# UniBwTAS/continuous_clustering

Hardware: AMD Instinct MI355X
Metric: Mpoints/s clustered (64-beam streams) (higher is better)
Workload: dtype f32

## Files before the change

### continuous_clustering_amd/csrc/cc_k_segment.h

```cpp
#pragma once


template<int RPL>
__device__ __forceinline__ void table_scan_tiles(const SP& p, const int R, const int ntiles, const int lane)
{
    float carry[RPL];
#pragma unroll
    for (int k = 0; k < RPL; k++)
    {
        const int row = k * 64 + lane;
        carry[k] = row < R ? p.curtab[row] : 0.f;
    }
    constexpr int U = 8;
    for (int t0 = 0; t0 < ntiles; t0 += U)
    {
        float v[U][RPL];
#pragma unroll
        for (int u = 0; u < U; u++)
#pragma unroll
            for (int k = 0; k < RPL; k++)
            {
                const int row = k * 64 + lane;
                v[u][k] = (row < R && t0 + u < ntiles) ? p.tabc[(size_t) (t0 + u) * R + row] : __builtin_nanf("");
            }
#pragma unroll
        for (int u = 0; u < U; u++)
#pragma unroll
            for (int k = 0; k < RPL; k++)
            {
                const int row = k * 64 + lane;
                if (row < R && t0 + u < ntiles)
                {
                    p.tabc[(size_t) (t0 + u) * R + row] = carry[k];
                    if (!(v[u][k] != v[u][k]))
                        carry[k] = v[u][k];
                }
            }
    }
#pragma unroll
    for (int k = 0; k < RPL; k++)
    {
        const int row = k * 64 + lane;
        if (row < R)
            p.curtab[row] = carry[k];
    }
}

template<int RPL>
__global__ __launch_bounds__(64 * TABLE_WAVES) void k_table(Geometry g, Planes P, StreamState* states, int first_stream, int slot)
{
    const int s = first_stream + blockIdx.x;
    const int lane = lane_id(), wave = uniform_i32((int) (threadIdx.x >> 6));
    StreamState* st = &states[s];
#ifdef CC_CHAIN2_PRIO
    __builtin_amdgcn_s_setprio(CC_CHAIN2_PRIO);
#endif
    if (threadIdx.x == 0)
        st->batch[slot].mode = st->assoc_mode;
    const long long seg_begin = st->batch[slot].seg_begin, seg_end = st->batch[slot].seg_end;
    if (seg_begin < 0 || seg_begin >= seg_end)
        return;
    if (st->batch[slot].fused)
        return;
    const SP p = stream_ptrs(P, g, s);
    const int R = g.num_rows, RC = g.ring_cols;
    const int ntiles = (int) ((seg_end - seg_begin + 63) >> 6);
    constexpr int U = 16;
    for (int t = wave; t < ntiles; t += TABLE_WAVES)
    {
        const long long c_lo = seg_begin + 64ll * t, c_hi = (c_lo + 64 < seg_end ? c_lo + 64 : seg_end);
        float last[RPL];
#pragma unroll
        for (int k = 0; k < RPL; k++)
            last[k] = __builtin_nanf("");
        int lc = (int) (c_lo % RC);
        for (long long c0 = c_lo; c0 < c_hi; c0 += U)
        {
            float cur[U][RPL], below[U][RPL];
#pragma unroll
            for (int u = 0; u < U; u++)
            {
#pragma unroll
                for (int k = 0; k < RPL; k++)
                {
                    const int row = k * 64 + lane;
                    cur[u][k] = below[u][k] = 0.f;
                    if (row < R && c0 + u < c_hi)
                    {
                        const size_t ci = (size_t) lc * R + row;
                        cur[u][k] = p.incl[ci];
                        below[u][k] = row + 1 < R ? p.incl[ci + 1] : 0.f;
                    }
                }
                lc = lc + 1 == RC ? 0 : lc + 1;
            }
#pragma unroll
            for (int u = 0; u < U; u++)
            {
                if (c0 + u >= c_hi)
                    break;
#pragma unroll
                for (int k = 0; k < RPL; k++)
                {
                    const float diff = cur[u][k] - below[u][k];
                    if (!(diff != diff))
                        last[k] = diff;
                }
            }
        }
#pragma unroll
        for (int k = 0; k < RPL; k++)
        {
            const int row = k * 64 + lane;
            if (row < R)
                p.tabc[(size_t) t * R + row] = last[k];
        }
    }
    __syncthreads();
    if (wave == 0)
        table_scan_tiles<RPL>(p, R, ntiles, lane);
}

__device__ __forceinline__ void ego_record(const StreamState* __restrict__ states, int first_stream, const cc_config& cfg, const double* __restrict__ poses,
                                           long long n, long long n_total, long long fbase, double* __restrict__ out, const int sl, const long long f)
{
    const double* A = states[first_stream + sl].robot_from_sensor;
    const double* T = poses + ((size_t) sl * (size_t) n_total + (size_t) fbase + (size_t) f) * 12;
    double ir[9], it[3];
    for (int i = 0; i < 3; i++)
        for (int j = 0; j < 3; j++)
            ir[i * 3 + j] = T[j * 4 + i];
    for (int i = 0; i < 3; i++)
        it[i] = ((-ir[i * 3 + 0]) * T[3] + (-ir[i * 3 + 1]) * T[7]) + (-ir[i * 3 + 2]) * T[11];
    double* o = out + ((size_t) sl * (size_t) n + (size_t) f) * EGO_STRIDE;
    for (int i = 0; i < 3; i++)
    {
        for (int j = 0; j < 3; j++)
            o[i * 3 + j] = (A[i * 4 + 0] * ir[0 * 3 + j] + A[i * 4 + 1] * ir[1 * 3 + j]) + A[i * 4 + 2] * ir[2 * 3 + j];
        o[9 + i] = ((A[i * 4 + 0] * it[0] + A[i * 4 + 1] * it[1]) + A[i * 4 + 2] * it[2]) + A[i * 4 + 3];
    }
    auto gram_dev = [](const double* m, const int stride) -> double
    {
        double dev = 0.;
        for (int a = 0; a < 3; a++)
            for (int b = 0; b < 3; b++)
            {
                double d = 0.;
                for (int k = 0; k < 3; k++)
                    d += m[k * stride + a] * m[k * stride + b];
                d -= a == b ? 1. : 0.;
                dev += d * d;
            }
        return __builtin_sqrt(dev);
    };
    const double dev_t = gram_dev(T, 4), dev_a = gram_dev(A, 4);
    auto mx2 = [](const float a, const float b) -> double
    {
        const double x = a, y = b;
        return x * x > y * y ? x * x : y * y;
    };
    const double box = __builtin_sqrt(mx2(cfg.length_ref_to_front_end_, cfg.length_ref_to_rear_end_) + mx2(cfg.width_ref_to_left_mirror_, cfg.width_ref_to_right_mirror_) +
                                      mx2(cfg.height_ref_to_maximum_, cfg.height_ref_to_ground_));
    const double at = __builtin_sqrt((A[3] * A[3] + A[7] * A[7]) + A[11] * A[11]);
    double skip = __builtin_inf();
    if (dev_t < 0.5 && dev_a < 0.5 && box == box && at == at)
    {
        const double sigma = __builtin_sqrt((1. - dev_t) * (1. - dev_a));
        const double delta = 2.4e-7 * ((__builtin_fabs(T[3]) + __builtin_fabs(T[7])) + __builtin_fabs(T[11])) + 1e-6;
        const double r = ((box + at) / sigma + delta) * 1.00001;
        const double r2 = r * r * 1.00001;
        float r2f = (float) r2;
        if ((double) r2f < r2)
            r2f = __builtin_bit_cast(float, __builtin_bit_cast(int, r2f) + 1);
        skip = r2f == r2f ? (double) r2f : __builtin_inf();
    }
    o[12] = skip;
}

__global__ __launch_bounds__(256) void k_ego(const StreamState* __restrict__ states, int first_stream, cc_config cfg, const double* __restrict__ poses,
                                             long long n, long long n_total, long long fbase, double* __restrict__ out)
{
    const long long f = (long long) blockIdx.x * 256 + threadIdx.x;
    if (f < n)
        ego_record(states, first_stream, cfg, poses, n, n_total, fbase, out, (int) blockIdx.y, f);
}


template<int RPL>
__global__ __launch_bounds__(64) void k_seg_pre(Geometry g, cc_config cfg, Planes P, StreamState* states, int first_stream, int slot,
                                                const double* __restrict__ poses, long long n_total, long long fbase,
                                                const double* __restrict__ ego, long long n_batch)
{
    const int sl = blockIdx.x;
    const int s = first_stream + sl;
    StreamState* st = &states[s];
    const long long seg_begin = st->batch[slot].seg_begin, seg_end = st->batch[slot].seg_end;
    if (seg_begin < 0 || seg_begin >= seg_end)
        return;
    if (st->batch[slot].fused)
        return;
    if (!st->has_robot_tf)
    {
        if (blockIdx.y == 0 && lane_id() == 0)
            raise_error(st, CC_ERR_NO_ROBOT_TRANSFORM, seg_begin, 0);
        return;
    }
    const SP p = stream_ptrs(P, g, s);
    const int R = g.num_rows, RC = g.ring_cols;
    const int lane = lane_id();

    const long long total = seg_end - seg_begin;
    const long long chunk_len = (total + SEGPRE_BLOCKS - 1) / SEGPRE_BLOCKS;
    const long long c_lo = seg_begin + chunk_len * (long long) blockIdx.y, c_hi = (c_lo + chunk_len < seg_end ? c_lo + chunk_len : seg_end);
    if (c_lo >= c_hi)
        return;
    const int NC = g.num_columns;
    int lc = (int) (c_lo % RC);
    long long rot = c_lo / NC;
    int cir = (int) (c_lo - rot * NC);
    long long pass = c_lo / RC;
    uint16_t a_tg[RPL];
    uint16_t n_tg[RPL];
    float n_dist[RPL], n_incaz[RPL];
    float4 n_rec[RPL];
    uint8_t n_inten[RPL];
    int n_trig = 0;
    auto load_tags = [&](const long long gcx, const int lcx)
    {
#pragma unroll
        for (int k = 0; k < RPL; k++)
        {
            const int row = k * 64 + lane;
            a_tg[k] = CELL_CLEARED;
            if (row < R && gcx < c_hi)
                a_tg[k] = p.gtag[(size_t) lcx * R + row];
        }
    };
    auto load_cells = [&](const long long gcx, const int lcx, const uint16_t tagx)
    {
#pragma unroll
        for (int k = 0; k < RPL; k++)
        {
            const int row = k * 64 + lane;
            n_dist[k] = n_incaz[k] = 0.f;
            n_inten[k] = 0;
            n_rec[k] = make_float4(__builtin_nanf(""), __builtin_nanf(""), __builtin_nanf(""), __builtin_nanf(""));
            if (row < R && gcx < c_hi)
            {
                const size_t ci = (size_t) lcx * R + row;
                n_dist[k] = p.dist[ci];
                if (n_tg[k] == tagx)
                {
                    n_rec[k] = p.sc_rec[ci];
                    n_incaz[k] = p.incaz[ci];
                    n_inten[k] = p.inten[ci];
                }
            }
        }
        if (gcx < c_hi)
            n_trig = p.trig[lcx];
    };
    load_tags(c_lo, lc);
    CazBase cb = caz_base_of_rotation(rot);
    long long cb_rot = rot;
    for (long long gc = c_lo; gc < c_hi; gc++, pass += (lc + 1 == RC ? 1 : 0), lc = (lc + 1 == RC ? 0 : lc + 1), rot += (cir + 1 == NC ? 1 : 0),
                   cir = (cir + 1 == NC ? 0 : cir + 1))
    {
        const size_t base = (size_t) lc * R;
        if (rot != cb_rot)
        {
            cb = caz_base_of_rotation(rot);
            cb_rot = rot;
        }
        const uint16_t tag = cell_tag(pass);
        {
#pragma unroll
            for (int k = 0; k < RPL; k++)
                n_tg[k] = a_tg[k];
            load_cells(gc, lc, tag);
            load_tags(gc + 1, lc + 1 == RC ? 0 : lc + 1);
        }
        const int trig = uniform_i32(n_trig);
        const double* T = poses + ((size_t) sl * (size_t) n_total + (size_t) fbase + (size_t) trig) * 12;
        const double* E = ego + ((size_t) sl * (size_t) n_batch + (size_t) trig) * EGO_STRIDE;
        const float spx = (float) T[3], spy = (float) T[7], spz = (float) T[11];

        float cx[RPL], cy[RPL], cz[RPL], dist[RPL], incl[RPL];
        bool empty_cell[RPL], overrun = false;
        int overrun_row = -1;
        long long overrun_gcol = -1;
#pragma unroll
        for (int k = 0; k < RPL; k++)
        {
            const int row = k * 64 + lane;
            dist[k] = incl[k] = __builtin_nanf("");
            cx[k] = cy[k] = cz[k] = 0.f;
            empty_cell[k] = false;
            if (row < R)
            {
                const uint16_t tg = n_tg[k];
                if (tg != tag && tg != CELL_CLEARED)
                {
                    overrun = true;
                    overrun_row = row;
                    overrun_gcol = gc - (long long) ((((unsigned) tag - (unsigned) tg) & 0x7fffu)) * RC;
                }
                empty_cell[k] = tg != tag;
                dist[k] = n_dist[k];
                cx[k] = n_rec[k].x;
                cy[k] = n_rec[k].y;
                cz[k] = n_rec[k].z;
                incl[k] = n_rec[k].w;
            }
        }
        if (__any(overrun))
        {
            const int worst = -wave_min_i32(-overrun_row);
            if (overrun_row == worst)
            {
                atomicMin((unsigned long long*) &st->overrun_col, (unsigned long long) gc);
                raise_error(st, CC_ERR_RING_OVERRUN, overrun_gcol, gc);
            }
            continue;
        }
        float x2[RPL], uz[RPL], w[RPL];
        int flags[RPL];
        seg_pre_cells<RPL>(cfg, R, lane, cx, cy, cz, dist, incl, n_inten, spx, spy, spz, E, x2, uz, w, flags);
        int kpos = 0x7fffffff, kneg = 0x7fffffff;
        bool any_empty = false;
#pragma unroll
        for (int k = 0; k < RPL; k++)
        {
            const int row = k * 64 + lane;
            if (row >= R)
                continue;
            const size_t ci = base + row;
            if (empty_cell[k])
                p.gtag[ci] = tag;
            if (flags[k] & SG_NAN)
                any_empty = true;
            else
                caz_key(n_incaz[k], kpos, kneg);
            p.sg_x2[ci] = x2[k];
            p.sg_uz[ci] = uz[k];
            p.sg_w[ci] = w[k];
            p.sg_flags[ci] = (uint8_t) flags[k];
        }
        const double min_az = column_min_caz(cb, kpos, kneg, any_empty, gc, g.az_width);
        if (lane == 0)
        {
            p.colg[lc] = gc;
            p.colminaz[lc] = min_az;
        }
    }
}

#ifndef CC_SEGSCAN_MIN_WAVES_PER_SIMD
#define CC_SEGSCAN_MIN_WAVES_PER_SIMD 2
#endif
constexpr int SEG_X2_RING = 16;
constexpr int SEG_CH = 16;
constexpr int SEG_FEW = 4;
__host__ __device__ inline int seg_pitch_f(int R)
{
    (void) R;
    return SEG_X2_RING + 1;
}
__host__ __device__ inline int seg_pitch_b(int R)
{
    return ((R + 3) & ~3) + 4;
}
__host__ __device__ inline bool seg_tiled(int R)
{
    return R >= SEG_CH && (R % SEG_CH) == 0;
}
__host__ inline size_t seg_scan_lds_bytes(int R)
{
    const size_t f = seg_tiled(R) ? (size_t) 4 * 64 * SEG_CH * 4 : (size_t) 64 * seg_pitch_f(R) * 4;
    return f + (size_t) 64 * seg_pitch_b(R);
}

enum
{
    SG_G_UNKNOWN = 0, SG_G_GROUND = 1, SG_G_OBSTACLE = 2, SG_G_EGO = 3, SG_G_FOG = 4,
    SG_D_WHITE = 0, SG_D_GRAY = 1, SG_D_ORANGE = 2, SG_D_GREEN = 3, SG_D_YELLOWGREEN = 4, SG_D_YELLOW = 5, SG_D_RED = 6, SG_D_DARKRED = 7,
    SG_D_VIOLET = 8, SG_D_LIGHTGRAY = 9
};

__global__ __launch_bounds__(64, CC_SEGSCAN_MIN_WAVES_PER_SIMD) void k_seg_scan(Geometry g, cc_config cfg, Planes P, StreamState* states, int first_stream, int slot)
{
    const int s = first_stream + blockIdx.x;
    StreamState* st = &states[s];
    const long long seg_begin = st->batch[slot].seg_begin, seg_end = st->batch[slot].seg_end;
    if (seg_begin < 0 || st->error != 0)
        return;
    const long long tile0 = seg_begin + (long long) blockIdx.y * 64;
    if (tile0 >= seg_end)
        return;
    const int ncols = (int) (seg_end - tile0 < 64 ? seg_end - tile0 : 64);
    const SP p = stream_ptrs(P, g, s);
    const int R = g.num_rows, RC = g.ring_cols;
    const int lane = lane_id();
    const int PF = seg_pitch_f(R), PB = seg_pitch_b(R);
    const bool tiled = seg_tiled(R);
    extern __shared__ __attribute__((aligned(16))) unsigned char smem[];
    float* l_x2 = (float*) smem;
    unsigned char* l_out = (unsigned char*) (l_x2 + (tiled ? 4 * 64 * SEG_CH : 64 * PF));

    const int lc0 = (int) (tile0 % RC);
    {
        const bool active = lane < ncols;
        const long long gc = tile0 + lane;
        int lcl = lc0 + lane;
        lcl = lcl >= RC ? lcl - RC : lcl;
        const float* gx = p.sg_x2 + (size_t) lcl * R;
        const float* gz = p.sg_uz + (size_t) lcl * R;
        const float* gw = p.sg_w + (size_t) lcl * R;
        const unsigned char* gf = p.sg_flags + (size_t) lcl * R;
        float4* g_rec = p.sc_rec + (size_t) lcl * R;
        float* g_incl = p.incl + (size_t) lcl * R;
        const float* tab_in = p.tabc + (size_t) blockIdx.y * R;
        unsigned char* oo = l_out + lane * PB;
        const float height_sensor_to_ground = -(float) st->robot_from_sensor[11] + cfg.height_ref_to_ground_;
        const bool chess_odd = cfg.ignore_points_in_chessboard_pattern && (gc & 1);
        const bool chess_even = cfg.ignore_points_in_chessboard_pattern && !(gc & 1);
        bool first_obstacle_detected = false, first_point_found = false;
        float lg2x = 0.f, lgz = height_sensor_to_ground;
        float pv2x = 0.f, pvz = 0.f;
        unsigned char previous_label = 0;
        auto row_step = [&](const int row, const int f, const float cur2x, const float cur2y, auto&& x2_below)
        {
            const bool valid = (f & (SG_NAN | SG_FOG | SG_EGO)) == 0;
            const bool first = valid & !first_point_found;
            const bool normal = valid & first_point_found;
            const bool ign = ((f & (SG_TOO_CLOSE | SG_INCL_IGNORE)) != 0) | ((row & 1) ? chess_even : chess_odd);
            const float h = cur2y - height_sensor_to_ground;
            const bool first_ground = (h > cfg.first_ring_as_ground_min_allowed_z_diff) & (h < cfg.first_ring_as_ground_max_allowed_z_diff);
            const float p2cx = cur2x - pv2x, p2cy = cur2y - pvz;
            const float slope_to_prev = p2cy / p2cx;
            const bool flat_prev = (ccm::absf(slope_to_prev) < cfg.max_slope) & (p2cx > 0) & ((cfg.use_terrain == 0) | (p2cx < 5));
            const float l2cx = cur2x - lg2x, l2cy = cur2y - lgz;
            const float slope_to_lg = l2cy / l2cx;
            const bool flat_lg = (ccm::absf(slope_to_lg) < cfg.max_slope) & (l2cx > 0);
            const bool no_terrain = cfg.use_terrain == 0;
            const bool green = !first_obstacle_detected & flat_prev;
            const bool yellowgreen = !green & no_terrain & first_obstacle_detected & flat_prev & flat_lg;
            const bool yellow = !green & !yellowgreen & no_terrain &
                                (ccm::absf(l2cx) < cfg.ground_because_close_to_last_certain_ground_max_dist_diff) &
                                (ccm::absf(l2cy) < cfg.ground_because_close_to_last_certain_ground_max_z_diff);
            const bool ground_n = green | yellowgreen | yellow;
            const unsigned d_n = green ? (unsigned) SG_D_GREEN : (yellowgreen ? (unsigned) SG_D_YELLOWGREEN : (yellow ? (unsigned) SG_D_YELLOW : (unsigned) SG_D_RED));
            const unsigned g_n = ground_n ? (unsigned) SG_G_GROUND : (unsigned) SG_G_OBSTACLE;
            const unsigned d_f = first_ground ? (unsigned) SG_D_GRAY : (unsigned) SG_D_ORANGE;
            const unsigned g_f = first_ground ? (unsigned) SG_G_GROUND : (unsigned) SG_G_OBSTACLE;
            unsigned g = first ? g_f : g_n, d = first ? d_f : d_n;
            g = (f & SG_EGO) ? (unsigned) SG_G_EGO : g;
            d = (f & SG_EGO) ? (unsigned) SG_D_VIOLET : d;
            g = (f & SG_FOG) ? (unsigned) SG_G_FOG : g;
            d = (f & SG_FOG) ? (unsigned) SG_D_LIGHTGRAY : d;
            g = (f & SG_NAN) ? (unsigned) SG_G_UNKNOWN : g;
            d = (f & SG_NAN) ? (unsigned) SG_D_WHITE : d;
            const bool red = normal & !ground_n;
            if (__any(red))
            {
                int below = row + 1;
                bool go = red & (below < R);
                while (__any(go))
                {
                    const int bi = go ? below : row + 1 < R ? row + 1 : row;
                    const unsigned bo = oo[bi];
                    const unsigned bg = bo & 7u, bd = (bo >> 3) & 15u;
                    const float xb = x2_below(bi, go);
                    const bool is_ground = bg == (unsigned) SG_G_GROUND;
                    const bool cont = go & ((bd == (unsigned) SG_D_YELLOW) |
                                            (is_ground & (ccm::absf(cur2x - xb) < cfg.obstacle_because_next_certain_obstacle_max_dist_diff)));
                    if (cont & is_ground)
                        oo[bi] = (unsigned char) ((bo & 0x80u) | SG_G_OBSTACLE | (SG_D_DARKRED << 3));
                    below += cont ? 1 : 0;
                    go = cont & (below < R);
                }
            }
            first_obstacle_detected = first ? !first_ground : (first_obstacle_detected | red);
            const bool keep_as_ground = normal & (green | yellowgreen) & (slope_to_prev > cfg.last_ground_point_slope_higher_than) &
                                        (ccm::absf(p2cx) < cfg.last_ground_point_distance_smaller_than) & (previous_label != SG_D_YELLOW);
            const bool new_lg = (first & first_ground) | keep_as_ground;
            lg2x = new_lg ? cur2x : lg2x;
            lgz = new_lg ? cur2y : lgz;
            pv2x = valid ? cur2x : pv2x;
            pvz = valid ? cur2y : pvz;
            previous_label = valid ? (unsigned char) d : previous_label;
            first_point_found |= valid;
            oo[row] = (unsigned char) (g | (d << 3) | ((valid & ign) ? 0x80u : 0u));
        };
        const unsigned long long le_mask = lane == 63 ? ~0ull : ((2ull << lane) - 1ull);
        const bool supplement = cfg.supplement_inclination_angle_for_nan_cells != 0;
        const bool step_filter = cfg.ignore_points_with_too_big_inclination_angle_diff != 0;
        float supp_below = __builtin_nanf("");
        bool below_nan = false;
        auto row_all = [&](const int row, const int f, const float cur2x, const float cur2y, const float wv, const float carry, auto&& x2_below,
                           auto&& stash) -> bool
        {
            const bool own = !(f & (SG_NAN | SG_PENDING));
            const unsigned long long m = __ballot(own) & le_mask;
            const int src = m ? 63 - __clzll((long long) m) : lane;
            const float got = __shfl(wv, src, 64);
            const float tab = m ? got : carry;
            const bool is_nan = (f & SG_NAN) != 0;
            const float supp = (supplement & (row < R - 1)) ? (below_nan ? supp_below : wv) + tab : __builtin_nanf("");
            if (is_nan & active)
            {
                g_rec[row] = make_float4(__builtin_nanf(""), __builtin_nanf(""), __builtin_nanf(""), supp);
                g_incl[row] = supp;
            }
            supp_below = is_nan ? supp : supp_below;
            below_nan = is_nan;
            const bool pend = ((f & (SG_PENDING | SG_NAN)) == SG_PENDING) & step_filter & (row < R - 1) & !(tab != tab);
            const float a = wv * tab;
            const bool in_range = (cfg.max_distance > 0.f) & (tab >= 0.f) & (tab < 0.05f) & (wv > 0.f) & (wv < 3.0e38f);
            const bool surely_not = in_range & (cfg.max_distance >= 1.01f * a);
            const bool surely = in_range & !surely_not & (cfg.max_distance * 1.000002f < a);
            const int fx = f | ((pend & surely) ? SG_INCL_IGNORE : 0);
            const bool need = pend & !surely_not & !surely;
            if (need)
                stash(tab);
            row_step(row, fx, cur2x, cur2y, x2_below);
            return need;
        };
        if (tiled && ncols <= SEG_FEW && 3 * SEG_FEW * R <= 4 * 64 * SEG_CH)
        {
            float* cx2 = l_x2;
            float* cuz = l_x2 + SEG_FEW * R;
            float* cw = l_x2 + 2 * SEG_FEW * R;
            for (int c = 0; c < ncols; c++)
            {
                int l = lc0 + c;
                l = l >= RC ? l - RC : l;
                for (int row = lane; row < R; row += 64)
                {
                    cx2[c * R + row] = p.sg_x2[(size_t) l * R + row];
                    cuz[c * R + row] = p.sg_uz[(size_t) l * R + row];
                    cw[c * R + row] = p.sg_w[(size_t) l * R + row];
                    l_out[c * PB + row] = p.sg_flags[(size_t) l * R + row];
                }
            }
            wave_lds_fence();
            asm volatile("s_waitcnt lgkmcnt(0)" ::: "memory");
            {
                const int lc_ = active ? lane : 0;
                const float* mx = cx2 + lc_ * R;
                const float* mz = cuz + lc_ * R;
                const float* mw = cw + lc_ * R;
                auto x2_below = [&](const int below, const bool wanted) -> float { (void) wanted; return mx[below]; };
                const float carry_lo = lane < R ? tab_in[lane] : 0.f, carry_hi = 64 + lane < R ? tab_in[64 + lane] : 0.f;
                auto carry_of = [&](const int row) -> float
                {
                    return __builtin_bit_cast(float, __builtin_amdgcn_readlane(__builtin_bit_cast(int, row < 64 ? carry_lo : carry_hi), row & 63));
                };
                for (int b = R - 4; b >= 0; b -= 4)
                {
                    const float4 a = *(const float4*) (mx + b);
                    const float4 c4 = *(const float4*) (mz + b);
                    const float4 w4 = *(const float4*) (mw + b);
                    const float x4[4] = {a.x, a.y, a.z, a.w}, z4[4] = {c4.x, c4.y, c4.z, c4.w}, ww[4] = {w4.x, w4.y, w4.z, w4.w};
                    const unsigned fw = active ? *(const unsigned*) (oo + b) : 0x01010101u * (unsigned) SG_NAN;
                    unsigned pend = 0;
#pragma unroll
                    for (int u = 3; u >= 0; u--)
                        if (row_all(b + u, (int) ((fw >> (8 * u)) & 0xffu), x4[u], z4[u], ww[u], carry_of(b + u), x2_below,
                                    [&](const float tab) { cuz[lc_ * R + b + u] = tab; }))
                            pend |= 1u << u;
                    if (__any(pend != 0))
                        for (int u = 0; u < 4; u++)
                            if (((pend >> u) & 1) && ccm::atan2f_exact(cfg.max_distance, mw[b + u]) < mz[b + u])
                                oo[b + u] |= 0x80;
                }
            }
        }
        else if (tiled)
        {
            float* t_uz = l_x2 + 2 * 64 * SEG_CH;
            float* t_w = l_x2 + 3 * 64 * SEG_CH;
            const int ld_c = lane >> 2, ld_q = lane & 3;
            int ld_off[4];
#pragma unroll
            for (int j = 0; j < 4; j++)
            {
                const int c = j * 16 + ld_c;
                int l = lc0 + c;
                l = l >= RC ? l - RC : l;
                ld_off[j] = c < ncols ? l * R : -1;
            }
            float4 nx[4], nz[4], nw[4];
            float ncarry = 0.f;
            auto load_chunk = [&](const int b)
            {
                ncarry = tab_in[b + (lane & 15)];
#pragma unroll
                for (int j = 0; j < 4; j++)
                {
                    nx[j] = nz[j] = nw[j] = make_float4(0.f, 0.f, 0.f, 0.f);
                    if (ld_off[j] >= 0)
                    {
                        nx[j] = *(const float4*) (p.sg_x2 + (size_t) ld_off[j] + b + ld_q * 4);
                        nz[j] = *(const float4*) (p.sg_uz + (size_t) ld_off[j] + b + ld_q * 4);
                        nw[j] = *(const float4*) (p.sg_w + (size_t) ld_off[j] + b + ld_q * 4);
                    }
                }
            };
            int b = R - SEG_CH;
            load_chunk(b);
            {
                const int npieces = R >> 4;
                for (int idx0 = lane; idx0 < 64 * npieces; idx0 += 4 * 64)
                {
                    uint4 v[4];
                    int dst[4];
#pragma unroll
                    for (int u = 0; u < 4; u++)
                    {
                        const int idx = idx0 + u * 64;
                        const int c = idx / npieces, piece = idx - c * npieces;
                        dst[u] = -1;
                        v[u] = make_uint4(0, 0, 0, 0);
                        if (idx < 64 * npieces && c < ncols)
                        {
                            int l = lc0 + c;
                            l = l >= RC ? l - RC : l;
                            v[u] = *(const uint4*) (p.sg_flags + (size_t) l * R + piece * 16);
                            dst[u] = c * PB + piece * 16;
                        }
                    }
#pragma unroll
                    for (int u = 0; u < 4; u++)
                        if (dst[u] >= 0)
                        {
                            unsigned* d = (unsigned*) (l_out + dst[u]);
                            d[0] = v[u].x, d[1] = v[u].y, d[2] = v[u].z, d[3] = v[u].w;
                        }
                }
            }
            auto piece_at = [](const int c, const int q) { return (c * 4 + (q ^ ((c >> 2) & 3))) * 4; };
            for (; b >= 0; b -= SEG_CH)
            {
                float* cx = l_x2 + ((b >> 4) & 1) * (64 * SEG_CH);
#pragma unroll
                for (int j = 0; j < 4; j++)
                {
                    const int c = j * 16 + ld_c;
                    *(float4*) (cx + piece_at(c, ld_q)) = nx[j];
                    *(float4*) (t_uz + piece_at(c, ld_q)) = nz[j];
                    *(float4*) (t_w + piece_at(c, ld_q)) = nw[j];
                }
                const int carry_bits = __builtin_bit_cast(int, ncarry);
                if (b >= SEG_CH)
                    load_chunk(b - SEG_CH);
                wave_lds_fence();
                {
                    auto x2_below = [&](const int below, const bool wanted) -> float
                    {
                        float v = l_x2[((below >> 4) & 1) * (64 * SEG_CH) + piece_at(lane, (below & 15) >> 2) + (below & 3)];
                        const bool deep = wanted & (below >= b + 2 * SEG_CH);
                        if (__any(deep))
                            if (deep)
                                v = gx[below];
                        return v;
                    };
                    unsigned pend = 0;
#pragma unroll 1
                    for (int q = 3; q >= 0; q--)
                    {
                        const int at = piece_at(lane, q);
                        const float4 a = *(const float4*) (cx + at);
                        const float4 c4 = *(const float4*) (t_uz + at);
                        const float4 w4 = *(const float4*) (t_w + at);
                        const float x4[4] = {a.x, a.y, a.z, a.w}, z4[4] = {c4.x, c4.y, c4.z, c4.w}, ww[4] = {w4.x, w4.y, w4.z, w4.w};
                        const unsigned fw = active ? *(const unsigned*) (oo + b + q * 4) : 0x01010101u * (unsigned) SG_NAN;
#pragma unroll
                        for (int u = 3; u >= 0; u--)
                            if (row_all(b + q * 4 + u, (int) ((fw >> (8 * u)) & 0xffu), x4[u], z4[u], ww[u],
                                        __builtin_bit_cast(float, __builtin_amdgcn_readlane(carry_bits, q * 4 + u)), x2_below,
                                        [&](const float tab) { t_uz[at + u] = tab; }))
                                pend |= 1u << (q * 4 + u);
                    }
                    if (__any(pend != 0))
                        for (int u = 0; u < SEG_CH; u++)
                        {
                            const int at = piece_at(lane, u >> 2) + (u & 3);
                            if (((pend >> u) & 1) && ccm::atan2f_exact(cfg.max_distance, t_w[at]) < t_uz[at])
                                oo[b + u] |= 0x80;
                        }
                }
                wave_lds_fence();
            }
        }
        else
        {
            float* x2 = l_x2 + lane * PF;
            const bool vec = (R & 7) == 0;
            float nx[8], nz[8], nw[8];
            unsigned nf0 = 0, nf1 = 0;
            auto load_chunk = [&](int b)
            {
                if (!active)
                {
                    nf0 = nf1 = 0x01010101u * (unsigned) SG_NAN;
#pragma unroll
                    for (int u = 0; u < 8; u++)
                        nx[u] = nz[u] = nw[u] = 0.f;
                }
                else if (vec)
                {
                    const float4 a0 = *(const float4*) (gx + b), a1 = *(const float4*) (gx + b + 4);
                    const float4 c0 = *(const float4*) (gz + b), c1 = *(const float4*) (gz + b + 4);
                    const float4 w0 = *(const float4*) (gw + b), w1 = *(const float4*) (gw + b + 4);
                    const uint2 ff = *(const uint2*) (gf + b);
                    nx[0] = a0.x, nx[1] = a0.y, nx[2] = a0.z, nx[3] = a0.w, nx[4] = a1.x, nx[5] = a1.y, nx[6] = a1.z, nx[7] = a1.w;
                    nz[0] = c0.x, nz[1] = c0.y, nz[2] = c0.z, nz[3] = c0.w, nz[4] = c1.x, nz[5] = c1.y, nz[6] = c1.z, nz[7] = c1.w;
                    nw[0] = w0.x, nw[1] = w0.y, nw[2] = w0.z, nw[3] = w0.w, nw[4] = w1.x, nw[5] = w1.y, nw[6] = w1.z, nw[7] = w1.w;
                    nf0 = ff.x;
                    nf1 = ff.y;
                }
                else
                {
                    nf0 = nf1 = 0;
#pragma unroll
                    for (int u = 0; u < 8; u++)
                    {
                        const int rr = b + u;
                        nx[u] = rr >= 0 ? gx[rr] : 0.f;
                        nz[u] = rr >= 0 ? gz[rr] : 0.f;
                        nw[u] = rr >= 0 ? gw[rr] : 0.f;
                        const unsigned f = rr >= 0 ? gf[rr] : (unsigned) SG_NAN;
                        if (u < 4)
                            nf0 |= f << (8 * u);
                        else
                            nf1 |= f << (8 * (u - 4));
                    }
                }
            };
            int b = R - 8;
            load_chunk(b);
            for (; b > -8; b -= 8)
            {
                float x8[8], z8[8], w8[8];
#pragma unroll
                for (int u = 0; u < 8; u++)
                {
                    x8[u] = nx[u];
                    z8[u] = nz[u];
                    w8[u] = nw[u];
                }
                const unsigned f0 = nf0, f1 = nf1;
                if (b - 8 > -8)
                    load_chunk(b - 8);
#pragma unroll
                for (int u = 0; u < 8; u++)
                    if (b + u >= 0)
                        x2[(b + u) & (SEG_X2_RING - 1)] = x8[u];
                auto x2_below = [&](const int below, const bool wanted) -> float
                {
                    float v = x2[below & (SEG_X2_RING - 1)];
                    const bool deep = wanted & (below >= b + SEG_X2_RING);
                    if (__any(deep))
                        if (deep)
                            v = gx[below];
                    return v;
                };
#pragma unroll
                for (int u = 7; u >= 0; u--)
                {
                    const int row = b + u;
                    if (row < 0)
                        break;
                    float tab_u = 0.f;
                    const bool pend = row_all(row, (int) (((u < 4 ? f0 : f1) >> (8 * (u & 3))) & 0xffu), x8[u], z8[u], w8[u], tab_in[row], x2_below,
                                              [&](const float tab) { tab_u = tab; });
                    if (__any(pend))
                        if (pend && ccm::atan2f_exact(cfg.max_distance, w8[u]) < tab_u)
                            oo[row] |= 0x80;
                }
            }
        }
    }
    __syncthreads();
    {
        int lc = lc0;
        for (int c = 0; c < ncols; c++)
        {
            for (int row = lane; row < R; row += 64)
            {
                const size_t ci = (size_t) lc * R + row;
                const unsigned char o = l_out[c * PB + row];
                constexpr unsigned long long GV = (unsigned long long) CC_GP_UNKNOWN | ((unsigned long long) CC_GP_GROUND << 8) |
                                                  ((unsigned long long) CC_GP_OBSTACLE << 16) | ((unsigned long long) CC_GP_EGO_VEHICLE << 24) |
                                                  ((unsigned long long) CC_GP_FOG << 32);
                constexpr unsigned long long DV0 = (unsigned long long) CC_DBG_WHITE | ((unsigned long long) CC_DBG_GRAY << 8) |
                                                   ((unsigned long long) CC_DBG_ORANGE << 16) | ((unsigned long long) CC_DBG_GREEN << 24) |
                                                   ((unsigned long long) CC_DBG_YELLOWGREEN << 32) | ((unsigned long long) CC_DBG_YELLOW << 40) |
                                                   ((unsigned long long) CC_DBG_RED << 48) | ((unsigned long long) CC_DBG_DARKRED << 56);
                constexpr unsigned DV1 = (unsigned) CC_DBG_VIOLET | ((unsigned) CC_DBG_LIGHTGRAY << 8);
                const unsigned dcode = (o >> 3) & 15;
                p.ground[ci] = (unsigned char) (GV >> (8 * (o & 7)));
                p.debug[ci] = (unsigned char) (dcode < 8 ? (DV0 >> (8 * dcode)) : (unsigned long long) (DV1 >> (8 * (dcode - 8))));
                const bool ign = (o & 7) != SG_G_OBSTACLE || (o & 0x80);
                p.ignored[ci] = ign ? 1 : 0;
            }
            lc = lc + 1 == RC ? 0 : lc + 1;
        }
    }
}

__device__ __forceinline__ void seg_small_body(const Geometry& g, const cc_config& cfg, const Planes& P, StreamState* states, int first_stream, int slot,
                                               const double* __restrict__ poses, long long n_total, long long fbase, const double* __restrict__ ego,
                                               long long n_batch, const int sl)
{
    const int s = first_stream + sl;
    StreamState* st = &states[s];
    const int lane = lane_id();
    if (lane == 0)
        st->batch[slot].mode = st->assoc_mode;
    const long long seg_begin = st->batch[slot].seg_begin, seg_end = st->batch[slot].seg_end;
    if (seg_begin < 0 || seg_begin >= seg_end || st->error != 0)
        return;
    if (!st->has_robot_tf)
    {
        if (lane == 0)
            raise_error(st, CC_ERR_NO_ROBOT_TRANSFORM, seg_begin, 0);
        return;
    }
    const SP p = stream_ptrs(P, g, s);
    const int R = g.num_rows, RC = g.ring_cols, NC = g.num_columns;
    const int row = lane;
    const bool inrow = row < R;
    const float height_sensor_to_ground = -(float) st->robot_from_sensor[11] + cfg.height_ref_to_ground_;
    const bool supplement = cfg.supplement_inclination_angle_for_nan_cells != 0;
    const bool step_filter = cfg.ignore_points_with_too_big_inclination_angle_diff != 0;
    const bool no_terrain = cfg.use_terrain == 0;
    const unsigned long long le = lane == 63 ? ~0ull : ((2ull << lane) - 1ull);
    const unsigned long long below = ~le, above = le >> 1;
    float tabrow = inrow ? p.curtab[row] : 0.f;
    int lc = (int) (seg_begin % RC);
    long long rot = seg_begin / NC;
    int cir = (int) (seg_begin - rot * NC);
    long long pass = seg_begin / RC;
    CazBase cb = caz_base_of_rotation(rot);
    for (long long gc = seg_begin; gc < seg_end; gc++)
    {
        const size_t ci = (size_t) lc * R + row;
        const uint16_t tag = cell_tag(pass);
        float cx[1] = {0.f}, cy[1] = {0.f}, cz[1] = {0.f}, dist[1] = {__builtin_nanf("")}, incl[1] = {__builtin_nanf("")};
        uint8_t inten[1] = {0};
        float incaz = 0.f;
        bool empty_cell = false, overrun = false;
        long long overrun_gcol = -1;
        if (inrow)
        {
            const uint16_t tg = p.gtag[ci];
            dist[0] = p.dist[ci];
            if (tg == tag)
            {
                const float4 r4 = p.sc_rec[ci];
                cx[0] = r4.x, cy[0] = r4.y, cz[0] = r4.z, incl[0] = r4.w;
                incaz = p.incaz[ci];
                inten[0] = p.inten[ci];
            }
            else
            {
                empty_cell = true;
                if (tg != CELL_CLEARED)
                {
                    overrun = true;
                    overrun_gcol = gc - (long long) ((((unsigned) tag - (unsigned) tg) & 0x7fffu)) * RC;
                }
            }
        }
        if (__any(overrun))
        {
            const int worst = -wave_min_i32(overrun ? -row : 1);
            if (overrun && row == worst)
            {
                atomicMin((unsigned long long*) &st->overrun_col, (unsigned long long) gc);
                raise_error(st, CC_ERR_RING_OVERRUN, overrun_gcol, gc);
            }
            break;
        }
        const int trig = uniform_i32(p.trig[lc]);
        const double* T = poses + ((size_t) sl * (size_t) n_total + (size_t) fbase + (size_t) trig) * 12;
        const double* E = ego + ((size_t) sl * (size_t) n_batch + (size_t) trig) * EGO_STRIDE;
        float x2a[1], uza[1], wa[1];
        int fla[1];
        seg_pre_cells<1>(cfg, R, lane, cx, cy, cz, dist, incl, inten, (float) T[3], (float) T[7], (float) T[11], E, x2a, uza, wa, fla);
        const int f = fla[0];
        const float cur2x = x2a[0], cur2y = uza[0], wv = wa[0];
        const bool is_nan = (f & SG_NAN) != 0;
        const bool own = !(f & (SG_NAN | SG_PENDING));
        const float tab = own ? wv : tabrow;
        tabrow = tab;
        float sincl = incl[0];
        bool done = !is_nan | !supplement | (row >= R - 1) | !inrow;
        while (__any(!done))
        {
            const float sb = __shfl_down(sincl, 1, 64);
            const int db = __shfl_down(done ? 1 : 0, 1, 64);
            if (!done && db)
            {
                sincl = sb + tab;
                done = true;
            }
        }
        bool ign = (f & (SG_TOO_CLOSE | SG_INCL_IGNORE)) != 0;
        {
            const bool pend = ((f & (SG_PENDING | SG_NAN)) == SG_PENDING) & step_filter & (row < R - 1) & !(tab != tab);
            const float a = wv * tab;
            const bool in_range = (cfg.max_distance > 0.f) & (tab >= 0.f) & (tab < 0.05f) & (wv > 0.f) & (wv < 3.0e38f);
            const bool surely_not = in_range & (cfg.max_distance >= 1.01f * a);
            const bool surely = in_range & !surely_not & (cfg.max_distance * 1.000002f < a);
            const bool need = pend & !surely_not & !surely;
            ign |= pend & surely;
            if (__any(need))
                if (need && ccm::atan2f_exact(cfg.max_distance, wv) < tab)
                    ign = true;
        }
        if (cfg.ignore_points_in_chessboard_pattern)
            ign |= ((gc & 1) != 0) != ((row & 1) != 0);
        const bool valid = inrow & ((f & (SG_NAN | SG_FOG | SG_EGO)) == 0);
        const unsigned long long V = __ballot(valid);
        const unsigned long long mb = V & below;
        const bool has_prev = mb != 0;
        const int pb = has_prev ? __ffsll((long long) mb) - 1 : lane;
        const bool first = valid & !has_prev, normal = valid & has_prev;
        const float pv2x = __shfl(cur2x, pb, 64), pvz = __shfl(cur2y, pb, 64);
        const float p2cx = cur2x - pv2x, p2cy = cur2y - pvz;
        const float slope_to_prev = p2cy / p2cx;
        const bool flat_prev = (ccm::absf(slope_to_prev) < cfg.max_slope) & (p2cx > 0) & (no_terrain | (p2cx < 5));
        const bool keep_geo = (slope_to_prev > cfg.last_ground_point_slope_higher_than) & (ccm::absf(p2cx) < cfg.last_ground_point_distance_smaller_than);
        const float h = cur2y - height_sensor_to_ground;
        const bool first_ground = (h > cfg.first_ring_as_ground_min_allowed_z_diff) & (h < cfg.first_ring_as_ground_max_allowed_z_diff);
        const bool first_obst = __any(first & !first_ground);
        unsigned d = first ? (first_ground ? (unsigned) SG_D_GRAY : (unsigned) SG_D_ORANGE)
                           : (normal ? (flat_prev ? (unsigned) SG_D_GREEN : (unsigned) SG_D_RED) : (unsigned) SG_D_WHITE);
        for (int round = 0; round <= R; round++)
        {
            const unsigned long long REDm = __ballot(normal & (d == (unsigned) SG_D_RED));
            const unsigned long long YELm = __ballot(normal & (d == (unsigned) SG_D_YELLOW));
            const bool fod = first_obst | ((REDm & below) != 0);
            const bool prev_yellow = has_prev & (((YELm >> pb) & 1ull) != 0);
            const bool upd = (first & first_ground) | (normal & ((d == (unsigned) SG_D_GREEN) | (d == (unsigned) SG_D_YELLOWGREEN)) & keep_geo & !prev_yellow);
            const unsigned long long ml = __ballot(upd) & below;
            const bool has_lg = ml != 0;
            const int lgrow = has_lg ? __ffsll((long long) ml) - 1 : lane;
            const float lgx = __shfl(cur2x, lgrow, 64), lgy = __shfl(cur2y, lgrow, 64);
            const float lg2x = has_lg ? lgx : 0.f, lgz = has_lg ? lgy : height_sensor_to_ground;
            const float l2cx = cur2x - lg2x, l2cy = cur2y - lgz;
            const float slope_to_lg = l2cy / l2cx;
            const bool flat_lg = (ccm::absf(slope_to_lg) < cfg.max_slope) & (l2cx > 0);
            const bool green = !fod & flat_prev;
            const bool yellowgreen = !green & no_terrain & fod & flat_prev & flat_lg;
            const bool yellow = !green & !yellowgreen & no_terrain & (ccm::absf(l2cx) < cfg.ground_because_close_to_last_certain_ground_max_dist_diff) &
                                (ccm::absf(l2cy) < cfg.ground_because_close_to_last_certain_ground_max_z_diff);
            const unsigned dn = normal ? (green ? (unsigned) SG_D_GREEN
                                                : (yellowgreen ? (unsigned) SG_D_YELLOWGREEN : (yellow ? (unsigned) SG_D_YELLOW : (unsigned) SG_D_RED)))
                                       : d;
            const bool changed = dn != d;
            d = dn;
            if (!__any(changed))
                break;
        }
        unsigned gl = (d == (unsigned) SG_D_ORANGE || d == (unsigned) SG_D_RED) ? (unsigned) SG_G_OBSTACLE : (unsigned) SG_G_GROUND;
        gl = valid ? gl : (unsigned) SG_G_UNKNOWN;
        if (f & SG_EGO)
        {
            gl = SG_G_EGO;
            d = SG_D_VIOLET;
        }
        if (f & SG_FOG)
        {
            gl = SG_G_FOG;
            d = SG_D_LIGHTGRAY;
        }
        if ((f & SG_NAN) || !inrow)
        {
            gl = SG_G_UNKNOWN;
            d = SG_D_WHITE;
        }
        {
            const unsigned long long REDm = __ballot(normal & (d == (unsigned) SG_D_RED));
            const unsigned long long RA = REDm & above;
            const bool has_ra = RA != 0;
            const int ra = has_ra ? 63 - __clzll((long long) RA) : lane;
            const float xr = __shfl(cur2x, ra, 64);
            const bool pass_test = has_ra & ((d == (unsigned) SG_D_YELLOW) |
                                             ((gl == (unsigned) SG_G_GROUND) & (ccm::absf(xr - cur2x) < cfg.obstacle_because_next_certain_obstacle_max_dist_diff)));
            const unsigned long long NP = __ballot(!pass_test);
            const unsigned long long le_ra = ra == 63 ? ~0ull : ((2ull << ra) - 1ull);
            const bool reached = has_ra & ((NP & le & ~le_ra) == 0);
            if (reached & (gl == (unsigned) SG_G_GROUND))
            {
                gl = SG_G_OBSTACLE;
                d = SG_D_DARKRED;
            }
        }
        if (inrow)
        {
            constexpr unsigned long long GV = (unsigned long long) CC_GP_UNKNOWN | ((unsigned long long) CC_GP_GROUND << 8) |
                                              ((unsigned long long) CC_GP_OBSTACLE << 16) | ((unsigned long long) CC_GP_EGO_VEHICLE << 24) |
                                              ((unsigned long long) CC_GP_FOG << 32);
            constexpr unsigned long long DV0 = (unsigned long long) CC_DBG_WHITE | ((unsigned long long) CC_DBG_GRAY << 8) |
                                               ((unsigned long long) CC_DBG_ORANGE << 16) | ((unsigned long long) CC_DBG_GREEN << 24) |
                                               ((unsigned long long) CC_DBG_YELLOWGREEN << 32) | ((unsigned long long) CC_DBG_YELLOW << 40) |
                                               ((unsigned long long) CC_DBG_RED << 48) | ((unsigned long long) CC_DBG_DARKRED << 56);
            constexpr unsigned DV1 = (unsigned) CC_DBG_VIOLET | ((unsigned) CC_DBG_LIGHTGRAY << 8);
            p.ground[ci] = (unsigned char) (GV >> (8 * gl));
            p.debug[ci] = (unsigned char) (d < 8 ? (DV0 >> (8 * d)) : (unsigned long long) (DV1 >> (8 * (d - 8))));
            p.ignored[ci] = (gl != (unsigned) SG_G_OBSTACLE || ign) ? 1 : 0;
            if (empty_cell)
                p.gtag[ci] = tag;
            if (is_nan)
            {
                p.sc_rec[ci] = make_float4(__builtin_nanf(""), __builtin_nanf(""), __builtin_nanf(""), sincl);
                p.incl[ci] = sincl;
            }
        }
        int kpos = 0x7fffffff, kneg = 0x7fffffff;
        if (inrow && !is_nan)
            caz_key(incaz, kpos, kneg);
        const double min_az = column_min_caz(cb, kpos, kneg, inrow && is_nan, gc, g.az_width);
        if (lane == 0)
        {
            p.colg[lc] = gc;
            p.colminaz[lc] = min_az;
        }
        lc = lc + 1 == RC ? 0 : lc + 1;
        pass += lc == 0 ? 1 : 0;
        cir = cir + 1 == NC ? 0 : cir + 1;
        if (cir == 0)
        {
            rot++;
            cb = caz_base_of_rotation(rot);
        }
    }
    if (inrow)
        p.curtab[row] = tabrow;
}

__global__ __launch_bounds__(64) void k_seg_small(Geometry g, cc_config cfg, Planes P, StreamState* states, int first_stream, int slot,
                                                  const double* __restrict__ poses, long long n_total, long long fbase, const double* __restrict__ ego,
                                                  long long n_batch)
{
    seg_small_body(g, cfg, P, states, first_stream, slot, poses, n_total, fbase, ego, n_batch, (int) blockIdx.x);
}
```

### continuous_clustering_amd/csrc/cc_math.h

```cpp
#pragma once
#include <stdint.h>

#if defined(__HIPCC__)
#define CCM_HD __host__ __device__ __forceinline__
#else
#define CCM_HD static inline
#endif

namespace ccm
{

CCM_HD int32_t f2i(float f)
{
    return __builtin_bit_cast(int32_t, f);
}
CCM_HD float i2f(int32_t i)
{
    return __builtin_bit_cast(float, i);
}
CCM_HD float absf(float x)
{
    return i2f(f2i(x) & 0x7fffffff);
}
CCM_HD float sqrt_rn(float x)
{
    return __builtin_sqrtf(x);
}

#if defined(__HIP_DEVICE_COMPILE__)
#define CCM_ANY(c) __any(c)
#else
#define CCM_ANY(c) (c)
#endif

CCM_HD float atanf_exact(float x)
{
    const float hi0 = 4.6364760399e-01f, hi1 = 7.8539812565e-01f, hi2 = 9.8279368877e-01f,
                hi3 = 1.5707962513e+00f;
    const float lo0 = 5.0121582440e-09f, lo1 = 3.7748947079e-08f, lo2 = 3.4473217170e-08f,
                lo3 = 7.5497894159e-08f;
    const float a0 = 3.3333334327e-01f, a1 = -2.0000000298e-01f, a2 = 1.4285714924e-01f,
                a3 = -1.1111110449e-01f, a4 = 9.0908870101e-02f, a5 = -7.6918758452e-02f,
                a6 = 6.6610731184e-02f, a7 = -5.8335702866e-02f, a8 = 4.9768779427e-02f,
                a9 = -3.6531571299e-02f, a10 = 1.6285819933e-02f;
    const int32_t hx = f2i(x);
    const int32_t ix = hx & 0x7fffffff;
    const float ax = absf(x);
    const bool r0 = ix < 0x3ee00000, r1 = ix < 0x3f300000, r2 = ix < 0x3f980000, r3 = ix < 0x401c0000;
    const float num = r0 ? x : (r1 ? 2.0f * ax - 1.0f : (r2 ? ax - 1.0f : (r3 ? ax - 1.5f : -1.0f)));
    const float den = r0 ? 1.0f : (r1 ? 2.0f + ax : (r2 ? ax + 1.0f : (r3 ? 1.0f + 1.5f * ax : ax)));
    const float hi = r1 ? hi0 : (r2 ? hi1 : (r3 ? hi2 : hi3));
    const float lo = r1 ? lo0 : (r2 ? lo1 : (r3 ? lo2 : lo3));
    const float t = num / den;
    const float z = t * t;
    const float w = z * z;
    const float s1 = z * (a0 + w * (a2 + w * (a4 + w * (a6 + w * (a8 + w * a10)))));
    const float s2 = w * (a1 + w * (a3 + w * (a5 + w * (a7 + w * a9))));
    const float small = t - t * (s1 + s2);
    const float r = hi - ((t * (s1 + s2) - lo) - t);
    float res = r0 ? small : (hx < 0 ? -r : r);
    res = ix < 0x31000000 ? x : res;
    if (CCM_ANY(ix >= 0x4c000000))
    {
        if (ix >= 0x4c000000)
            res = ix > 0x7f800000 ? x + x : (hx > 0 ? hi3 + lo3 : -hi3 - lo3);
    }
    return res;
}

CCM_HD float atan2f_special(float y, float x)
{
    const float tiny = 1.0e-30f, pi_o_4 = 7.8539818525e-01f, pi_o_2 = 1.5707963705e+00f, pi = 3.1415927410e+00f;
    const int32_t hx = f2i(x), hy = f2i(y);
    const int32_t ix = hx & 0x7fffffff, iy = hy & 0x7fffffff;
    if (ix > 0x7f800000 || iy > 0x7f800000)
        return x + y;
    if (hx == 0x3f800000)
        return atanf_exact(y);
    const int m = ((hy >> 31) & 1) | ((hx >> 30) & 2);
    if (iy == 0)
    {
        if (m < 2)
            return y;
        return m == 2 ? pi + tiny : -pi - tiny;
    }
    if (ix == 0)
        return hy < 0 ? -pi_o_2 - tiny : pi_o_2 + tiny;
    if (ix == 0x7f800000)
    {
        if (iy == 0x7f800000)
        {
            switch (m)
            {
                case 0:
                    return pi_o_4 + tiny;
                case 1:
                    return -pi_o_4 - tiny;
                case 2:
                    return 3.0f * pi_o_4 + tiny;
                default:
                    return -3.0f * pi_o_4 - tiny;
            }
        }
        switch (m)
        {
            case 0:
                return 0.0f;
            case 1:
                return -0.0f;
            case 2:
                return pi + tiny;
            default:
                return -pi - tiny;
        }
    }
    return hy < 0 ? -pi_o_2 - tiny : pi_o_2 + tiny;
}

CCM_HD float atan2f_exact(float y, float x)
{
    const float pi_o_2 = 1.5707963705e+00f, pi = 3.1415927410e+00f, pi_lo = -8.7422776573e-08f;
    const int32_t hx = f2i(x), hy = f2i(y);
    const int32_t ix = hx & 0x7fffffff, iy = hy & 0x7fffffff;
    const bool special = (ix >= 0x7f800000) | (iy >= 0x7f800000) | (hx == 0x3f800000) | (iy == 0) | (ix == 0);
    const int m = ((hy >> 31) & 1) | ((hx >> 30) & 2);
    const int32_t k = (iy - ix) >> 23;
    const float za = atanf_exact(absf(y / x));
    const float z = k > 60 ? pi_o_2 + 0.5f * pi_lo : ((hx < 0 && k < -60) ? 0.0f : za);
    const float zz = z - pi_lo;
    float res = m == 0 ? z : (m == 1 ? i2f(f2i(z) ^ (int32_t) 0x80000000) : (m == 2 ? pi - zz : zz - pi));
    if (CCM_ANY(special))
    {
        if (special)
            res = atan2f_special(y, x);
    }
    return res;
}

CCM_HD float asinf_exact(float x)
{
    const float pio2_hi = 1.57079637050628662109375f, pio2_lo = -4.37113900018624283e-8f,
                pio4_hi = 0.785398185253143310546875f;
    const float p0 = 1.666675248e-1f, p1 = 7.495297643e-2f, p2 = 4.547037598e-2f, p3 = 2.417951451e-2f,
                p4 = 4.216630880e-2f;
    const int32_t hx = f2i(x);
    const int32_t ix = hx & 0x7fffffff;
    const float t0 = x * x;
    const float w0 = t0 * (p0 + t0 * (p1 + t0 * (p2 + t0 * (p3 + t0 * p4))));
    float res = ix < 0x32000000 ? x : x + x * w0;
    if (__builtin_expect(CCM_ANY(ix >= 0x3f000000), 0))
    {
        if (ix >= 0x3f000000)
        {
            if (ix == 0x3f800000)
                res = x * pio2_hi + x * pio2_lo;
            else if (ix > 0x3f800000)
                res = (x - x) / (x - x);
            else
            {
                float w = 1.0f - absf(x);
                float t = w * 0.5f;
                float p = t * (p0 + t * (p1 + t * (p2 + t * (p3 + t * p4))));
                const float s = sqrt_rn(t);
                if (ix >= 0x3F79999A)
                {
                    t = pio2_hi - (2.0f * (s + s * p) - pio2_lo);
                }
                else
                {
                    w = i2f(f2i(s) & (int32_t) 0xfffff000);
                    const float c = (t - w * w) / (s + w);
                    const float r = p;
                    p = 2.0f * s * r - (pio2_lo - 2.0f * c);
                    const float q = pio4_hi - 2.0f * w;
                    t = pio4_hi - (p - q);
                }
                res = hx > 0 ? t : -t;
            }
        }
    }
    return res;
}

}
```

Baseline: 17890.

## Use approximate reciprocal slope tests with exact-division fallback; vectorize label output

Slope comparisons in the ground-segmentation row step now use a hardware reciprocal estimate checked against widened threshold bounds. Only when the estimate falls in the uncertainty band (or is out of range) does the wave compute the exact IEEE divisions, which keeps results bit-identical while avoiding two full divisions per row in the common case. The final label conversion in the tiled path is also vectorized: it packs four bytes per word, maps them through byte-permute lookup tables, and writes uint4 stores instead of per-byte stores. The risks are extra branches and register pressure, plus the ncols*npieces loop assuming R is a multiple of 16.

```diff
diff --git a/continuous_clustering_amd/csrc/cc_k_segment.h b/continuous_clustering_amd/csrc/cc_k_segment.h
--- a/continuous_clustering_amd/csrc/cc_k_segment.h
+++ b/continuous_clustering_amd/csrc/cc_k_segment.h
@@ -428,6 +428,15 @@
         float lg2x = 0.f, lgz = height_sensor_to_ground;
         float pv2x = 0.f, pvz = 0.f;
         unsigned char previous_label = 0;
+        auto scalar_f32 = [](const float v)
+        {
+            float s_;
+            asm volatile("v_readfirstlane_b32 %0, %1" : "=s"(s_) : "v"(v));
+            return s_;
+        };
+        ccm::RatioBound slope_max = ccm::ratio_bound_abs_lt(cfg.max_slope), slope_keep = ccm::ratio_bound_gt(cfg.last_ground_point_slope_higher_than);
+        slope_max.sure_lo = scalar_f32(slope_max.sure_lo), slope_max.sure_hi = scalar_f32(slope_max.sure_hi);
+        slope_keep.sure_lo = scalar_f32(slope_keep.sure_lo), slope_keep.sure_hi = scalar_f32(slope_keep.sure_hi);
         auto row_step = [&](const int row, const int f, const float cur2x, const float cur2y, auto&& x2_below)
         {
             const bool valid = (f & (SG_NAN | SG_FOG | SG_EGO)) == 0;
@@ -437,11 +446,23 @@
             const float h = cur2y - height_sensor_to_ground;
             const bool first_ground = (h > cfg.first_ring_as_ground_min_allowed_z_diff) & (h < cfg.first_ring_as_ground_max_allowed_z_diff);
             const float p2cx = cur2x - pv2x, p2cy = cur2y - pvz;
-            const float slope_to_prev = p2cy / p2cx;
-            const bool flat_prev = (ccm::absf(slope_to_prev) < cfg.max_slope) & (p2cx > 0) & ((cfg.use_terrain == 0) | (p2cx < 5));
             const float l2cx = cur2x - lg2x, l2cy = cur2y - lgz;
-            const float slope_to_lg = l2cy / l2cx;
-            const bool flat_lg = (ccm::absf(slope_to_lg) < cfg.max_slope) & (l2cx > 0);
+            const float qe_prev = p2cy * __builtin_amdgcn_rcpf(p2cx), qe_lg = l2cy * __builtin_amdgcn_rcpf(l2cx);
+            bool sure_a, sure_b, sure_c;
+            bool prev_below_max = ccm::ratio_abs_lt(qe_prev, slope_max, sure_a);
+            bool prev_above_keep = ccm::ratio_gt(qe_prev, slope_keep, sure_b);
+            bool lg_below_max = ccm::ratio_abs_lt(qe_lg, slope_max, sure_c);
+            const bool open = valid & !(ccm::ratio_in_window(p2cx, qe_prev) & ccm::ratio_in_window(l2cx, qe_lg) & sure_a & sure_b & sure_c);
+            if (__any(open))
+            {
+                const float slope_to_prev = p2cy / p2cx;
+                const float slope_to_lg = l2cy / l2cx;
+                prev_below_max = open ? ccm::absf(slope_to_prev) < cfg.max_slope : prev_below_max;
+                prev_above_keep = open ? slope_to_prev > cfg.last_ground_point_slope_higher_than : prev_above_keep;
+                lg_below_max = open ? ccm::absf(slope_to_lg) < cfg.max_slope : lg_below_max;
+            }
+            const bool flat_prev = prev_below_max & (p2cx > 0) & ((cfg.use_terrain == 0) | (p2cx < 5));
+            const bool flat_lg = lg_below_max & (l2cx > 0);
             const bool no_terrain = cfg.use_terrain == 0;
             const bool green = !first_obstacle_detected & flat_prev;
             const bool yellowgreen = !green & no_terrain & first_obstacle_detected & flat_prev & flat_lg;
@@ -481,7 +502,7 @@
                 }
             }
             first_obstacle_detected = first ? !first_ground : (first_obstacle_detected | red);
-            const bool keep_as_ground = normal & (green | yellowgreen) & (slope_to_prev > cfg.last_ground_point_slope_higher_than) &
+            const bool keep_as_ground = normal & (green | yellowgreen) & prev_above_keep &
                                         (ccm::absf(p2cx) < cfg.last_ground_point_distance_smaller_than) & (previous_label != SG_D_YELLOW);
             const bool new_lg = (first & first_ground) | keep_as_ground;
             lg2x = new_lg ? cur2x : lg2x;
@@ -783,6 +804,47 @@
         }
     }
     __syncthreads();
+    constexpr unsigned long long GV = (unsigned long long) CC_GP_UNKNOWN | ((unsigned long long) CC_GP_GROUND << 8) |
+                                      ((unsigned long long) CC_GP_OBSTACLE << 16) | ((unsigned long long) CC_GP_EGO_VEHICLE << 24) |
+                                      ((unsigned long long) CC_GP_FOG << 32);
+    constexpr unsigned long long DV0 = (unsigned long long) CC_DBG_WHITE | ((unsigned long long) CC_DBG_GRAY << 8) |
+                                       ((unsigned long long) CC_DBG_ORANGE << 16) | ((unsigned long long) CC_DBG_GREEN << 24) |
+                                       ((unsigned long long) CC_DBG_YELLOWGREEN << 32) | ((unsigned long long) CC_DBG_YELLOW << 40) |
+                                       ((unsigned long long) CC_DBG_RED << 48) | ((unsigned long long) CC_DBG_DARKRED << 56);
+    constexpr unsigned DV1 = (unsigned) CC_DBG_VIOLET | ((unsigned) CC_DBG_LIGHTGRAY << 8);
+    if (tiled)
+    {
+        const int npieces = R >> 4;
+        auto convert = [&](const unsigned w, unsigned& gl, unsigned& dl, unsigned& ig)
+        {
+            const unsigned gcode = w & 0x07070707u, dcode = (w >> 3) & 0x0f0f0f0fu, dlow = dcode & 0x07070707u;
+            gl = __builtin_amdgcn_perm((unsigned) (GV >> 32), (unsigned) GV, gcode);
+            const unsigned d07 = __builtin_amdgcn_perm((unsigned) (DV0 >> 32), (unsigned) DV0, dlow);
+            const unsigned d89 = __builtin_amdgcn_perm(0u, DV1, dlow);
+            const unsigned high = ((dcode >> 3) & 0x01010101u) * 0xffu;
+            dl = (d07 & ~high) | (d89 & high);
+            const unsigned not_obstacle = ((gcode ^ (0x01010101u * (unsigned) SG_G_OBSTACLE)) + 0x07070707u) >> 3;
+            ig = (not_obstacle | (w >> 7)) & 0x01010101u;
+        };
+        for (int idx = lane; idx < ncols * npieces; idx += 64)
+        {
+            const int c = idx / npieces, piece = idx - c * npieces;
+            int l = lc0 + c;
+            l = l >= RC ? l - RC : l;
+            const unsigned* src = (const unsigned*) (l_out + c * PB + piece * 16);
+            const unsigned w0 = src[0], w1 = src[1], w2 = src[2], w3 = src[3];
+            uint4 gl, dl, ig;
+            convert(w0, gl.x, dl.x, ig.x);
+            convert(w1, gl.y, dl.y, ig.y);
+            convert(w2, gl.z, dl.z, ig.z);
+            convert(w3, gl.w, dl.w, ig.w);
+            const size_t ci = (size_t) l * R + piece * 16;
+            *(uint4*) (p.ground + ci) = gl;
+            *(uint4*) (p.debug + ci) = dl;
+            *(uint4*) (p.ignored + ci) = ig;
+        }
+    }
+    else
     {
         int lc = lc0;
         for (int c = 0; c < ncols; c++)
@@ -791,14 +853,6 @@
             {
                 const size_t ci = (size_t) lc * R + row;
                 const unsigned char o = l_out[c * PB + row];
-                constexpr unsigned long long GV = (unsigned long long) CC_GP_UNKNOWN | ((unsigned long long) CC_GP_GROUND << 8) |
-                                                  ((unsigned long long) CC_GP_OBSTACLE << 16) | ((unsigned long long) CC_GP_EGO_VEHICLE << 24) |
-                                                  ((unsigned long long) CC_GP_FOG << 32);
-                constexpr unsigned long long DV0 = (unsigned long long) CC_DBG_WHITE | ((unsigned long long) CC_DBG_GRAY << 8) |
-                                                   ((unsigned long long) CC_DBG_ORANGE << 16) | ((unsigned long long) CC_DBG_GREEN << 24) |
-                                                   ((unsigned long long) CC_DBG_YELLOWGREEN << 32) | ((unsigned long long) CC_DBG_YELLOW << 40) |
-                                                   ((unsigned long long) CC_DBG_RED << 48) | ((unsigned long long) CC_DBG_DARKRED << 56);
-                constexpr unsigned DV1 = (unsigned) CC_DBG_VIOLET | ((unsigned) CC_DBG_LIGHTGRAY << 8);
                 const unsigned dcode = (o >> 3) & 15;
                 p.ground[ci] = (unsigned char) (GV >> (8 * (o & 7)));
                 p.debug[ci] = (unsigned char) (dcode < 8 ? (DV0 >> (8 * dcode)) : (unsigned long long) (DV1 >> (8 * (dcode - 8))));
diff --git a/continuous_clustering_amd/csrc/cc_math.h b/continuous_clustering_amd/csrc/cc_math.h
--- a/continuous_clustering_amd/csrc/cc_math.h
+++ b/continuous_clustering_amd/csrc/cc_math.h
@@ -25,6 +25,49 @@
 CCM_HD float sqrt_rn(float x)
 {
     return __builtin_sqrtf(x);
+}
+
+struct RatioBound
+{
+    float sure_lo, sure_hi;
+    bool usable;
+};
+CCM_HD bool ratio_threshold_usable(float t)
+{
+    return (t == 0.0f) | ((absf(t) >= 0x1p-60f) & (absf(t) <= 0x1p60f));
+}
+CCM_HD RatioBound ratio_bound_abs_lt(float t)
+{
+    RatioBound b;
+    b.usable = ratio_threshold_usable(t);
+    b.sure_lo = b.usable ? t * (1.0f - 0x1p-20f) : __builtin_nanf("");
+    b.sure_hi = b.usable ? t * (1.0f + 0x1p-20f) : __builtin_nanf("");
+    return b;
+}
+CCM_HD RatioBound ratio_bound_gt(float t)
+{
+    const float u = t * (1.0f - 0x1p-20f), v = t * (1.0f + 0x1p-20f);
+    RatioBound b;
+    b.usable = ratio_threshold_usable(t);
+    b.sure_lo = b.usable ? (u < v ? u : v) : __builtin_nanf("");
+    b.sure_hi = b.usable ? (u < v ? v : u) : __builtin_nanf("");
+    return b;
+}
+CCM_HD bool ratio_in_window(float b, float qe)
+{
+    return (absf(b) >= 0x1p-40f) & (absf(b) < 0x1p40f) & (absf(qe) >= 0x1p-80f);
+}
+CCM_HD bool ratio_abs_lt(float qe, const RatioBound& t, bool& sure)
+{
+    const bool yes = absf(qe) < t.sure_lo, no = absf(qe) >= t.sure_hi;
+    sure = yes | no;
+    return yes;
+}
+CCM_HD bool ratio_gt(float qe, const RatioBound& t, bool& sure)
+{
+    const bool yes = qe > t.sure_hi, no = qe <= t.sure_lo;
+    sure = yes | no;
+    return yes;
 }
 
 #if defined(__HIP_DEVICE_COMPILE__)
```

Result: slower. 17520 (-2.1%).
